# yangdongchao/RSTnet

Measured on AMD Instinct MI355X. Metric: codec+LM audio frames/sec (24 kHz, 12.5 Hz tokens) at batch=1 and batch=64; RVQ code-index exact-match, higher is better.
Workload: dtype f32 (large GEMMs: operands as three bf16 planes, six bf16 matrix-instruction products per fp32 product, f32 accumulate); 1 GPU; MimiCodec encode->RVQ(8x2048x256)->decode, BASELINE.json configs[1]; batch_per_gpu=64, weights=random-init (rstnet_amd.synth seed 0), parallelism=replica x1, utterances sharded, RCCL weight broadcast only

## Files before the change

### include/rstnet_hip.h

```cpp
#ifndef RSTNET_HIP_H
#define RSTNET_HIP_H

#include <stdint.h>

#ifdef __cplusplus
extern "C" {
#endif

#define RST_OK 0
#define RST_ERR_INVALID_ARG (-1)
#define RST_ERR_UNSUPPORTED (-2)
#define RST_ERR_LAUNCH (-3)

#define RST_ACT_NONE 0
#define RST_ACT_ELU 1
#define RST_ACT_GELU 1
#define RST_ACT_ELU_OUT 2
#define RST_PAD_ZERO 0
#define RST_PAD_REPLICATE 1

typedef void* rst_stream_t;

int rst_version(void);
const char* rst_last_error(void);
// ... 51 lines not shown

int rst_gemv_f32(const float* x, const float* ln_gamma, const float* ln_beta, float ln_eps, const float* w, const float* bias,
                 const float* res, const float* scale, float* y, int B, int N, int K, int act_out, rst_stream_t stream);

int rst_layernorm_f32(const float* x, const float* gamma, const float* beta, float* y, int64_t rows, int D, float eps,
                      rst_stream_t stream);

int rst_rope_split_f32(const float* qkv, float* q, float* k, float* v, const int64_t* pos_dev, int64_t pos0, int B,
                       int T, int H, int D, int cap, int ring, int rope, float rope_coef, rst_stream_t stream);

int rst_attention_f32(const float* q, const float* k, const float* v, float* out, const int64_t* pos_dev, int64_t pos0,
                      int B, int T, int H, int D, int cap, int ring, int context, rst_stream_t stream);

int rst_rope_table_f32(float* table, int T, int D, float rope_coef, int64_t pos0, rst_stream_t stream);
int rst_attention_qkv_f32(const float* qkv, const float* rope_table, float* out, int B, int T, int H, int D, int context,
                          rst_stream_t stream);

int rst_rvq_pack_f32(const float* emb, float* packed, float* e2, int n_codes, int D, rst_stream_t stream);

int rst_rvq_search_f32(const float* x, const float* emb, const float* packed, const float* e2, int64_t* codes,
                       float* dist, uint64_t* keys, int M, int F, int ldx, int D, int n_codes, int L, int n_groups,
                       const int* group_begin, const int* group_count, rst_stream_t stream);

int rst_rvq_chain_slot_elems(int M, int n_codes, int L);
int rst_rvq_chain_supported(int M, int n_codes, int L, int D, int n_groups);
int rst_rvq_search_chain_f32(const float* x, const float* emb, const float* packed, const float* e2, int64_t* codes, float* dist,
                             uint64_t* slots, uint32_t* status, int M, int F, int ldx, int D, int n_codes, int L, int n_groups,
                             const int* group_begin, const int* group_count, rst_stream_t stream);

int rst_rvq_gather_f32(const int64_t* codes, const float* emb, float* out, int M, int F, int D, int n_codes, int L,
                       int n_groups, const int* group_begin, const int* group_count, rst_stream_t stream);

int rst_convtr_depthwise_f32(const float* x, const float* hist, const float* w, float* y, int B, int T_in, int C,
                             int Kw, int stride, rst_stream_t stream);

int rst_act_f32(const float* x, float* y, int64_t n, int act, rst_stream_t stream);

int rst_transpose_f32(const float* x, float* y, int B, int R, int C, rst_stream_t stream);

int rst_mask_tail_f32(float* x, const int32_t* lengths, int B, int T, int C, int mode, rst_stream_t stream);

int rst_hist_update_f32(const float* x, const float* hist_in, float* hist_out, int B, int T_in, int P_in, int P_out,
                        int C, rst_stream_t stream);

int rst_hist_update_batch_f32(const float* const* x, float* const* hist, const int* T_in, const int* P, const int* C, int n, int B,
                              rst_stream_t stream);
// ... 125 lines not shown
```

### rstnet_amd/_lib.py

```python
from __future__ import annotations

import ctypes as C
import os
from typing import Optional

_HERE = os.path.dirname(os.path.abspath(__file__))
LIB_PATH = os.path.join(_HERE, "librstnet_hip.so")

_p = C.c_void_p
_i = C.c_int
_l = C.c_int64
_f = C.c_float

SIGNATURES = {
    "rst_build_id": [_p, _i],
    "rst_gemm_win_split_plan": [_l, _i, _i],
    "rst_gemm_win_split_tiles": [_l, _i],
    "rst_gemm_win_f32": [_p, _p, _p, _p, _p, _p, _p, _i, _i, _i, _i, _i, _i, _i, _i, _i, _l, _i, _i, _i, _i, _p, _p, _p],
    "rst_gemm_win_b3_supported": [_i, _i, _i, _i, _i, _i, _i, _i, _i, _l, _i],
    "rst_gemm_win_b3_weight_elems": [_i, _i],
    "rst_gemm_win_b3_pack_weight": [_p, _p, _i, _i, _p],
    "rst_gemm_win_b3_f32": [_p, _p, _p, _p, _p, _p, _p, _p, _i, _i, _i, _i, _i, _i, _i, _i, _i, _l, _i, _i, _i, _p],
    "rst_conv1d_causal_f32": [_p, _p, _p, _p, _p, _p, _i, _i, _i, _i, _i, _i, _i, _i, _i, _i, _p],
    "rst_convtr1d_causal_f32": [_p, _p, _p, _p, _p, _i, _i, _i, _i, _i, _i, _i, _i, _p],
    "rst_seanet_resblock_supported": [_i, _i, _i, _i, _i, _i, _i],
    "rst_seanet_resblock_f32": [_p] * 11 + [_i] * 8 + [_p],
    "rst_seanet_resblock_b3_supported": [_i] * 9,
    "rst_seanet_resblock_b3_weight_elems": [_i],
    "rst_seanet_resblock_b3_pack": [_p, _p, _p, _p, _i, _i, _i, _i, _p],
    "rst_seanet_resblock_b3_f32": [_p] * 8 + [_i] * 8 + [_p],
    "rst_linear_f32": [_p, _p, _p, _p, _p, _p, _l, _i, _i, _i, _p],
    "rst_layernorm_f32": [_p, _p, _p, _p, _l, _i, _f, _p],
    "rst_rope_split_f32": [_p, _p, _p, _p, _p, _l, _i, _i, _i, _i, _i, _i, _i, _f, _p],
    "rst_attention_f32": [_p, _p, _p, _p, _p, _l, _i, _i, _i, _i, _i, _i, _i, _p],
    "rst_rope_table_f32": [_p, _i, _i, _f, _l, _p],
    "rst_attention_qkv_f32": [_p, _p, _p, _i, _i, _i, _i, _i, _p],
    "rst_rvq_pack_f32": [_p, _p, _p, _i, _i, _p],
    "rst_rvq_search_f32": [_p, _p, _p, _p, _p, _p, _p, _i, _i, _i, _i, _i, _i, _i, C.POINTER(_i), C.POINTER(_i), _p],
    "rst_rvq_chain_slot_elems": [_i, _i, _i],
    "rst_rvq_chain_supported": [_i, _i, _i, _i, _i],
    "rst_rvq_search_chain_f32": [_p, _p, _p, _p, _p, _p, _p, _p, _i, _i, _i, _i, _i, _i, _i, C.POINTER(_i), C.POINTER(_i), _p],
    "rst_rvq_gather_f32": [_p, _p, _p, _i, _i, _i, _i, _i, _i, C.POINTER(_i), C.POINTER(_i), _p],
    "rst_convtr_depthwise_f32": [_p, _p, _p, _p, _i, _i, _i, _i, _i, _p],
    "rst_act_f32": [_p, _p, _l, _i, _p],
    "rst_transpose_f32": [_p, _p, _i, _i, _i, _p],
    "rst_hist_update_f32": [_p, _p, _p, _i, _i, _i, _i, _i, _p],
    "rst_hist_update_batch_f32": [C.POINTER(_p), C.POINTER(_p), C.POINTER(_i), C.POINTER(_i), C.POINTER(_i), _i, _i, _p],
    "rst_skinny_f32_pack_weight": [_p, _p, _i, _i, _p],
    "rst_skinny_f32_pack_win": [_p, _p, _p, _i, _i, _i, _i, _i, _i, _i, _i, _l, _i, _p],
    "rst_skinny_f32_pack_ln": [_p, _p, _p, _f, _p, _i, _i, _p],
    "rst_skinny_f32_split_plan": [_i, _i, _i],
    "rst_gemm_skinny_f32": [_p, _p, _p, _p, _p, _p, _i, _i, _i, _i, _i, _i, _p, _p, _i, _p],
    "rst_linear_few_rows_f32": [_p, _i, _p, _p, _p, _p, _p, _i, _i, _i, _i, _i, _i, _p, _p, _i, _p],
    "rst_mask_tail_f32": [_p, _p, _i, _i, _i, _i, _p],
    "rst_codec_transformer_workspace_bytes": [_i, _i, _i],
    "rst_codec_transformer_supported": [_i, _i, _i, _i, _i, _i, _i],
    "rst_codec_transformer_frame": [C.POINTER(_p)] * 12 + [_p, _p, _p, _p, _p] + [_i] * 9 + [_f, _f, _p],
    "rst_gemv_f32": [_p, _p, _p, _f, _p, _p, _p, _p, _p, _i, _i, _i, _i, _p],
    "rst_gemv_bf16_f32": [_p, _p, _p, _p, _p, _p, _i, _i, _i, _i, _i, _i, _f, _i, _p],
    "rst_quant_rows_fp8": [_p, _p, _p, _i, _i, _p],
    "rst_gemv_fp8w_supported": [_i, _i, _i],
# ... 88 lines not shown
```

### rstnet_amd/codec/quantization.py

```python
from __future__ import annotations

from typing import List, Optional, Tuple

import torch
from torch import nn

from .. import ops
from .conv import _PackedCache, _to_ncl, _to_nlc


class EuclideanCodebook(nn.Module):

    def __init__(self, dim: int, codebook_size: int, decay: float = 0.99, epsilon: float = 1e-5,
                 threshold_usage_ratio: float = 0.1, replaced_usage_ratio: float = 1.0, check_unused_every: int = 5):
        super().__init__()
        self.dim, self.codebook_size, self.epsilon, self.decay = dim, codebook_size, epsilon, decay
        self.register_buffer("_initialized", torch.tensor([False], dtype=torch.float))
        self.register_buffer("cluster_usage", torch.ones(codebook_size))
        self.register_buffer("embedding_sum", torch.zeros(codebook_size, dim))
        self._emb = _PackedCache()
        self._emb_tables = _PackedCache()

    def _load_from_state_dict(self, state_dict, prefix, *args, **kwargs) -> None:
        for old, new in (("inited", "_initialized"), ("cluster_size", "cluster_usage"), ("embed_avg", "embedding_sum"),
# ... 143 lines not shown
    def __init__(self, *, n_q: int = 8, no_quantization_rate: float = 0.0, no_quantization_mode: str = "same",
                 n_q_semantic: int = 1, **kwargs):
        super().__init__()
        assert n_q > n_q_semantic, f"Number of quantizers {n_q} must be larger than the number of semantic quantizers {n_q_semantic}."
        self.max_n_q = n_q
        self.n_q_semantic = n_q_semantic
        self.n_q_acoustic = n_q - n_q_semantic
        kwargs.pop("q_dropout", None)
        kwargs.pop("generator_seed", None)
        self.rvq_first = ResidualVectorQuantizer(n_q=n_q_semantic, force_projection=True, q_dropout=False, **kwargs)
        self.rvq_rest = ResidualVectorQuantizer(n_q=n_q - n_q_semantic, codebook_offset=1, force_projection=True, **kwargs)
        self._fused = _PackedCache()

    def _fused_tables(self):
        f, r = self.rvq_first, self.rvq_rest
        embs = [l.embedding for l in f.vq.layers] + [l.embedding for l in r.vq.layers]
        params = (f.input_proj.weight, r.input_proj.weight, f.output_proj.weight, r.output_proj.weight) + tuple(embs)

        def build():
            w_in = torch.cat([f.input_proj.weight[:, :, 0], r.input_proj.weight[:, :, 0]], 0).float().contiguous()
            w_out = torch.cat([f.output_proj.weight[:, :, 0], r.output_proj.weight[:, :, 0]], 1).float().contiguous()
            emb = torch.stack(embs).contiguous()
            packed, e2 = ops.rvq_pack(emb)
            return w_in, w_out, emb, packed, e2
        return self._fused.get(params, build)

    def _groups(self, n_total: Optional[int] = None) -> List[Tuple[int, int]]:
        ns = self.rvq_first.n_q
        nr = self.rvq_rest.n_q if n_total is None else n_total - ns
        return [(0, ns), (self.n_q_semantic, nr)]

    def encode_nlc(self, z: torch.Tensor) -> torch.Tensor:
        B, F, C = z.shape
        K = self.rvq_first.n_q + self.rvq_rest.n_q
        if F == 0:
            return torch.empty((B, K, 0), device=z.device, dtype=torch.int64)
        w_in, _, emb, packed, e2 = self._fused_tables()
        x = ops.linear(z.reshape(B * F, C), w_in)
        codes = ops.rvq_search(x, emb, packed, e2, B, F, self._groups())
        return codes if K == codes.shape[1] else codes[:, :K].contiguous()

    def decode_nlc(self, codes: torch.Tensor) -> torch.Tensor:
        B, K, F = codes.shape
        _, w_out, emb, _, _ = self._fused_tables()
        if K < self.max_n_q:
            pad = torch.zeros(B, self.max_n_q - K, F, device=codes.device, dtype=torch.int64)
            codes = torch.cat([codes, pad], 1)
        q = ops.rvq_gather(codes.contiguous(), emb, self._groups(K))
        return ops.linear(q, w_out).view(B, F, -1)

    def forward(self, x: torch.Tensor, frame_rate: int, semantic_features: Optional[torch.Tensor] = None):
        raise NotImplementedError("training forward (losses, distillation) is out of scope; use encode / decode")

    def encode(self, x: torch.Tensor) -> torch.Tensor:
        return self.encode_nlc(_to_nlc(x))

    def decode(self, codes: torch.Tensor) -> torch.Tensor:
        return _to_ncl(self.decode_nlc(codes))

    @property
    def total_codebooks(self) -> int:
        return self.rvq_first.max_n_q + self.rvq_rest.max_n_q

    @property
    def num_codebooks(self) -> int:
        return self.rvq_first.num_codebooks + self.rvq_rest.num_codebooks

# ... 25 lines not shown
```

### rstnet_amd/csrc/capi.hip

```cpp
#include "../../include/rstnet_hip.h"
#include "rst_kernels.h"
#include <stdarg.h>
#include <stdio.h>

static thread_local char g_err[512] = "";

void rst_set_error(const char* fmt, ...) {
    va_list ap;
    va_start(ap, fmt);
    vsnprintf(g_err, sizeof(g_err), fmt, ap);
    va_end(ap);
}

int rst_check_launch(const char* what) {
    const hipError_t e = hipGetLastError();
    if (e != hipSuccess) {
        rst_set_error("%s: launch failed: %s", what, hipGetErrorString(e));
        return RST_ERR_LAUNCH;
    }
    return RST_OK;
}

extern "C" {

int rst_version(void) { return 125; }
const char* rst_last_error(void) { return g_err; }

#ifndef RST_SRC_SHA
#define RST_SRC_SHA "unknown"
#endif
int rst_build_id(char* out, int n) {
    static const char id[] = RST_SRC_SHA;
    if (!out || n < (int)sizeof(id)) return RST_ERR_INVALID_ARG;
    for (int i = 0; i < (int)sizeof(id); ++i) out[i] = id[i];
    return (int)sizeof(id) - 1;
}

static int gemm_win_common(const float* x, const float* hist, const float* w, const uint16_t* w3, const float* bias, const float* res,
                           const float* scale, float* y, int B, int T_in, int T_out, int C, int K, int N, int S, int P,
                           int pad_mode, int64_t x_bstride, int ldy, int act_in, int act_out, int split_k, float* ws,
                           uint32_t* counters, rst_stream_t stream) {
    RST_REQUIRE(ldy >= N, "gemm_win: ldy (%d) < N (%d)", ldy, N);
    RST_REQUIRE(act_in == 0 || act_in == 1, "gemm_win: unknown act_in %d", act_in);
    RST_REQUIRE(act_out >= 0 && act_out <= 2, "gemm_win: unknown act_out %d", act_out);
    RST_REQUIRE(pad_mode == 0 || pad_mode == 1, "gemm_win: unknown pad_mode %d", pad_mode);
    GemmWinParams p;
    p.x = x; p.hist = hist; p.w = w; p.bias = bias; p.res = res; p.scale = scale; p.y = y;
    p.B = B; p.T_in = T_in; p.T_out = T_out; p.C = C; p.K = K; p.N = N; p.S = S; p.P = P;
// ... 140 lines not shown
    p.row_stride = 3 * H * D; p.rope_tab = rope_table;
    return rst_launch_attention(p, (hipStream_t)stream);
}

int rst_rvq_pack_f32(const float* emb, float* packed, float* e2, int n_codes, int D, rst_stream_t stream) {
    return rst_launch_rvq_pack(emb, packed, e2, n_codes, D, (hipStream_t)stream);
}

int rst_rvq_search_f32(const float* x, const float* emb, const float* packed, const float* e2, int64_t* codes,
                       float* dist, uint64_t* keys, int M, int F, int ldx, int D, int n_codes, int L, int n_groups,
                       const int* group_begin, const int* group_count, rst_stream_t stream) {
    RST_REQUIRE(n_groups >= 1 && n_groups <= 2 && group_begin && group_count, "rvq_search: bad groups");
    RvqSearchParams p;
    p.x = x; p.emb = emb; p.packed = packed; p.e2 = e2; p.codes = (long*)codes; p.dist = dist;
    p.M = M; p.F = F; p.ldx = ldx; p.D = D; p.n_codes = n_codes; p.L = L; p.n_groups = n_groups;
    for (int g = 0; g < 2; ++g) {
        p.group_begin[g] = g < n_groups ? group_begin[g] : 0;
        p.group_count[g] = g < n_groups ? group_count[g] : 0;
        RST_REQUIRE(p.group_begin[g] >= 0 && p.group_count[g] >= 0 && p.group_begin[g] + p.group_count[g] <= L,
                    "rvq_search: group %d out of range", g);
    }
    if (keys) return rst_launch_rvq_search_small(p, (unsigned long long*)keys, (hipStream_t)stream);
    return rst_launch_rvq_search(p, (hipStream_t)stream);
}

int rst_rvq_chain_supported(int M, int n_codes, int L, int D, int n_groups) { return rst_rvq_chain_supported_impl(M, n_codes, L, D, n_groups); }

int rst_rvq_chain_slot_elems(int M, int n_codes, int L) {
    if (M <= 0 || n_codes <= 0 || L <= 0 || (long)L * ((M + 31) / 32 * 32) * rst_rvq_chain_slices(n_codes) > 0x7fffffffL) return -1;
    return L * ((M + 31) / 32 * 32) * rst_rvq_chain_slices(n_codes);
}

int rst_rvq_search_chain_f32(const float* x, const float* emb, const float* packed, const float* e2, int64_t* codes, float* dist,
                             uint64_t* slots, uint32_t* status, int M, int F, int ldx, int D, int n_codes, int L, int n_groups,
                             const int* group_begin, const int* group_count, rst_stream_t stream) {
    RST_REQUIRE(n_groups >= 1 && n_groups <= 2 && group_begin && group_count, "rvq_search_chain: bad groups");
    RvqSearchParams p;
    p.x = x; p.emb = emb; p.packed = packed; p.e2 = e2; p.codes = (long*)codes; p.dist = dist;
    p.M = M; p.F = F; p.ldx = ldx; p.D = D; p.n_codes = n_codes; p.L = L; p.n_groups = n_groups;
    for (int g = 0; g < 2; ++g) {
        p.group_begin[g] = g < n_groups ? group_begin[g] : 0;
        p.group_count[g] = g < n_groups ? group_count[g] : 0;
        RST_REQUIRE(p.group_begin[g] >= 0 && p.group_count[g] >= 0 && p.group_begin[g] + p.group_count[g] <= L,
                    "rvq_search_chain: group %d out of range", g);
    }
    return rst_launch_rvq_search_chain(p, (unsigned long long*)slots, (unsigned*)status, (hipStream_t)stream);
// ... 491 lines not shown
```

### rstnet_amd/csrc/rst_kernels.h

```cpp
#pragma once
#include "rst_common.h"

struct GemmWinParams {
    const float* x;
    const float* hist;
    const float* w;
    const float* bias;
    const float* res;
    const float* scale;
    float* y;
    int B, T_in, T_out;
    int C;
    int K, N;
    int S;
    int P;
    int pad_mode;
    long x_bstride;
    int ldy;
    int act_in;
    int act_out;
    int split_k;
    float* ws;
    unsigned* counters;
    const short* w3;
// ... 125 lines not shown
    const long* pos_dev;
    long pos0;
    int B, T, H, D, cap;
    int ring;
    int context;
    int row_stride;
    const float* rope_tab;
};
int rst_launch_attention(const AttentionParams& p, hipStream_t stream);
int rst_launch_rope_table(float* tab, int T, int D, float rope_coef, long pos0, hipStream_t stream);

int rst_launch_rvq_pack(const float* emb, float* packed, float* e2, int n_codes, int D, hipStream_t stream);
struct RvqSearchParams {
    const float* x;
    const float* emb;
    const float* packed;
    const float* e2;
    long* codes;
    float* dist;
    int M, F, ldx, D, n_codes, L;
    int n_groups;
    int group_begin[2];
    int group_count[2];
};
int rst_launch_rvq_search(const RvqSearchParams& p, hipStream_t stream);
int rst_launch_rvq_search_small(const RvqSearchParams& p, unsigned long long* keys, hipStream_t stream);
int rst_rvq_chain_slices(int n_codes);
int rst_rvq_chain_supported_impl(int M, int n_codes, int L, int D, int n_groups);
int rst_launch_rvq_search_chain(const RvqSearchParams& p, unsigned long long* slots, unsigned* status, hipStream_t stream);
struct RvqGatherParams {
    const long* codes;
    const float* emb;
    float* out;
    int M, F, D, n_codes, L, n_groups;
    int group_begin[2];
    int group_count[2];
};
int rst_launch_rvq_gather(const RvqGatherParams& p, hipStream_t stream);

struct GemvParams {
    const float* x;
    const float* alpha;
    const float* beta;
    const void* w;
    const float* res;
    const float* bias;
    const float* scale;
    float* y;
// ... 250 lines not shown
```

### rstnet_amd/csrc/rvq.hip

```cpp
#include "rst_common.h"
#include "rst_kernels.h"
#include <math.h>

namespace {

constexpr int FR = 32;
constexpr int NW = 8;

__device__ __forceinline__ int pk_off(int k) { return (k >> 3) * 8 + (k & 1) * 4 + ((k >> 1) & 3); }

__global__ __launch_bounds__(256) void rvq_pack_kernel(const float* __restrict__ emb, float* __restrict__ packed,
                                                       float* __restrict__ e2, int n_codes, int D) {
    const long total = (long)n_codes * D;
    for (long idx = (long)blockIdx.x * 256 + threadIdx.x; idx < total; idx += (long)gridDim.x * 256) {
        const int k = (int)(idx % D);
        const long code = idx / D;
        packed[((long)(k >> 3) * n_codes + code) * 8 + (k & 1) * 4 + ((k >> 1) & 3)] = emb[idx];
    }
    for (long code = (long)blockIdx.x * 256 + threadIdx.x; code < n_codes; code += (long)gridDim.x * 256) {
        float s = 0.f;
        for (int k = 0; k < D; ++k) s = fmaf(emb[code * D + k], emb[code * D + k], s);
        e2[code] = s;
    }
}
// ... 97 lines not shown
        __syncthreads();
        if (tid < FR) {
            float bs = red_s[tid];
            int bi = red_i[tid];
            for (int w = 1; w < NW; ++w) {
                const float s = red_s[w * FR + tid];
                const int i = red_i[w * FR + tid];
                if (s < bs || (s == bs && i < bi)) { bs = s; bi = i; }
            }
            if (bi < 0 || bi >= p.n_codes) bi = 0;
            win[tid] = bi;
            const int m = m0 + tid;
            if (m < p.M) {
                const int b = m / p.F, f = m - b * p.F;
                p.codes[((long)b * p.L + lvl) * p.F + f] = bi;
                if (p.dist) p.dist[(long)lvl * p.M + m] = bs;
            }
        }
        __syncthreads();
        if (li + 1 < p.group_count[g]) {
            for (int idx = tid; idx < FR * D; idx += 64 * NW) {
                const int f = idx / D, k = idx - f * D;
                r_pk[f * LD + pk_off(k)] -= emb[(long)win[f] * D + k];
            }
        }
        __syncthreads();
    }
}

__device__ __forceinline__ unsigned long long rvq_key(float score, int code) {
    unsigned u = __float_as_uint(score);
    u = (u & 0x80000000u) ? ~u : (u | 0x80000000u);
    return ((unsigned long long)u << 32) | (unsigned)code;
}

__global__ __launch_bounds__(256) void rvq_level_kernel(const RvqSearchParams p, unsigned long long* __restrict__ keys, int step) {
    extern __shared__ __attribute__((aligned(16))) float smem[];
    const int D = p.D, LD = D + 4;
    float* r_pk = smem;
    int* prev = reinterpret_cast<int*>(r_pk + FR * LD);
    const int tid = threadIdx.x, lane = tid & 63, wave = tid >> 6;
    const int j = lane & 31, h = lane >> 5;
    const int g = blockIdx.y;
    if (step >= p.group_count[g]) return;
    const int lvl = p.group_begin[g] + step;
    const int m0 = blockIdx.z * FR;
// ... 303 lines not shown
}

int rst_launch_rvq_search(const RvqSearchParams& p, hipStream_t stream) {
    if (p.M == 0) return RST_OK;
    RST_REQUIRE(p.x && p.emb && p.packed && p.e2 && p.codes, "rvq_search: null pointer");
    RST_REQUIRE(p.M >= 0 && p.F > 0 && p.D > 0 && p.D % 8 == 0 && p.n_codes > 0 && p.n_codes % 32 == 0,
                "rvq_search: need D %% 8 == 0 and n_codes %% 32 == 0 (D=%d n_codes=%d)", p.D, p.n_codes);
    RST_REQUIRE(p.n_groups >= 1 && p.n_groups <= 2, "rvq_search: n_groups must be 1 or 2");
    RST_REQUIRE(p.M % p.F == 0, "rvq_search: M (%d) is not a multiple of F (%d)", p.M, p.F);
    if (p.M == 0) return RST_OK;
    const size_t lds = ((size_t)FR * (p.D + 4) + p.n_codes + 2 * NW * FR + FR) * sizeof(float);
    RST_REQUIRE(lds <= 160 * 1024, "rvq_search: D=%d n_codes=%d needs %zu bytes of LDS", p.D, p.n_codes, lds);
    static RstOncePerDevice attr_once;
    if (attr_once.first()) {
        (void)hipFuncSetAttribute(reinterpret_cast<const void*>(rvq_search_kernel<32>), hipFuncAttributeMaxDynamicSharedMemorySize, 160 * 1024);
        (void)hipFuncSetAttribute(reinterpret_cast<const void*>(rvq_search_kernel<0>), hipFuncAttributeMaxDynamicSharedMemorySize, 160 * 1024);
    }
    const dim3 grid((p.M + FR - 1) / FR, p.n_groups);
    if (p.D == 256) hipLaunchKernelGGL(rvq_search_kernel<32>, grid, dim3(64 * NW), lds, stream, p);
    else hipLaunchKernelGGL(rvq_search_kernel<0>, grid, dim3(64 * NW), lds, stream, p);
    return rst_check_launch("rvq_search");
}

int rst_launch_rvq_search_small(const RvqSearchParams& p, unsigned long long* keys, hipStream_t stream) {
    if (p.M == 0) return RST_OK;
    RST_REQUIRE(p.x && p.emb && p.packed && p.e2 && p.codes && keys, "rvq_search_small: null pointer");
    RST_REQUIRE(p.F > 0 && p.D > 0 && p.D % 8 == 0 && p.n_codes > 0 && p.n_codes % 32 == 0 && p.M % p.F == 0 &&
                    p.n_groups >= 1 && p.n_groups <= 2,
                "rvq_search_small: need D %% 8 == 0 and n_codes %% 32 == 0 (D=%d n_codes=%d)", p.D, p.n_codes);
    const size_t lds = ((size_t)FR * (p.D + 4) + 16 * FR) * sizeof(float);
    int steps = 0;
    for (int g = 0; g < p.n_groups; ++g) steps = p.group_count[g] > steps ? p.group_count[g] : steps;
    const dim3 grid((p.n_codes + 127) / 128, p.n_groups, (p.M + FR - 1) / FR);
    RST_REQUIRE(steps <= 16, "rvq_search_small: at most 16 levels per group (got %d)", steps);
    for (int s = 0; s < steps; ++s) {
        hipLaunchKernelGGL(rvq_level_kernel, grid, dim3(256), lds, stream, p, keys, s);
        const int rc = rst_check_launch("rvq_level");
        if (rc) return rc;
    }
    long g = ((long)p.L * p.M + 255) / 256;
    hipLaunchKernelGGL(rvq_finalize_kernel, dim3((unsigned)(g > 64 ? 64 : g)), dim3(256), 0, stream, p, keys);
    return rst_check_launch("rvq_finalize");
}

int rst_rvq_chain_slices(int n_codes) { return (n_codes + 127) / 128; }

// ... 39 lines not shown
```

### rstnet_amd/ops.py

```python
from __future__ import annotations

import ctypes as C
import functools
import math
from typing import NamedTuple, Optional, Sequence, Tuple

import torch

from . import _lib

ACT_NONE, ACT_ELU, ACT_GELU = 0, 1, 1
ACT_ELU_OUT = 2
PAD_ZERO, PAD_REPLICATE = 0, 1


PROFILE = None


class _profiled:
    __slots__ = ("row", "prof", "e0", "e1")

    def __init__(self, name: str, flops: float, nbytes: int, shape: tuple):
        self.row = (name, flops, nbytes, shape)

# ... 545 lines not shown
               groups: Sequence[Tuple[int, int]], return_dist: bool = False):
    for t, n in ((x, "x"), (emb, "emb"), (packed, "packed"), (e2, "e2")):
        _chk(t, n)
    L, n_codes, D = emb.shape
    M = B * F
    assert x.shape == (M, len(groups) * D), (tuple(x.shape), M, len(groups), D)
    covered = sorted(l for g0, n in groups for l in range(g0, g0 + n)) == list(range(L))
    codes = (torch.empty if covered else torch.zeros)(B, L, F, device=x.device, dtype=torch.int64)
    dist = torch.zeros(L, M, device=x.device, dtype=torch.float32) if return_dist else None
    keys = None
    if 0 < M <= 64 and RVQ_CHAIN and n_codes % 128 == 0 and depth_frame_enabled(x.device) and \
            _rvq_chain_supported(_device_index(x.device), M, n_codes, L, D, len(groups)):
        n_slots = int(_lib.lib().rst_rvq_chain_slot_elems(M, n_codes, L))
        sc = _scratch(_rvq_slots, x.device, (L, M, n_codes),
                      lambda: (torch.full((n_slots,), -1, device=x.device, dtype=torch.int64), new_persistent_status(x.device)))
        _lib.check(_lib.lib().rst_rvq_search_chain_f32(_ptr(x), _ptr(emb), _ptr(packed), _ptr(e2), _ptr(codes), _ptr(dist), _ptr(sc[0]), _ptr(sc[1]),
                                                       M, max(F, 1), x.shape[1], D, n_codes, L, len(groups), *_group_arrays(groups),
                                                       _stream()))
        return (codes, dist) if return_dist else codes
    if 0 < M <= 64:
        keys = _scratch(_rvq_keys, x.device, (L, M), lambda: torch.full((L, M), -1, device=x.device, dtype=torch.int64))
    _lib.check(_lib.lib().rst_rvq_search_f32(_ptr(x), _ptr(emb), _ptr(packed), _ptr(e2), _ptr(codes), _ptr(dist), _ptr(keys), M, max(F, 1),
                                             x.shape[1], D, n_codes, L, len(groups), *_group_arrays(groups), _stream()))
    return (codes, dist) if return_dist else codes


@_on_tensor_device
def rvq_gather(codes: torch.Tensor, emb: torch.Tensor, groups: Sequence[Tuple[int, int]]) -> torch.Tensor:
    _chk(codes, "codes", torch.int64)
    _chk(emb, "emb")
    B, L, F = codes.shape
    _, n_codes, D = emb.shape
    out = torch.empty(B * F, len(groups) * D, device=codes.device, dtype=torch.float32)
    _lib.check(_lib.lib().rst_rvq_gather_f32(_ptr(codes), _ptr(emb), _ptr(out), B * F, max(F, 1), D, n_codes, L, len(groups),
                                             *_group_arrays(groups), _stream()))
    return out


@_on_tensor_device
def convtr_depthwise(x: torch.Tensor, w: torch.Tensor, stride: int, hist: Optional[torch.Tensor] = None) -> torch.Tensor:
    for t, n in ((x, "x"), (w, "w"), (hist, "hist")):
        _chk(t, n)
    B, T, Cc = x.shape
    out = torch.empty(B, T * stride, Cc, device=x.device, dtype=torch.float32)
    _lib.check(_lib.lib().rst_convtr_depthwise_f32(_ptr(x), _ptr(hist), _ptr(w), _ptr(out), B, T, Cc, w.shape[1], stride,
                                                   _stream()))
# ... 1037 lines not shown
```

Measured before the change: 197,800 frames/s.

## Add bf16-plane filtered RVQ search with exact fp32 rescoring of survivors

```diff
diff --git a/include/rstnet_hip.h b/include/rstnet_hip.h
--- a/include/rstnet_hip.h
+++ b/include/rstnet_hip.h
@@ -97,6 +97,11 @@
                        float* dist, uint64_t* keys, int M, int F, int ldx, int D, int n_codes, int L, int n_groups,
                        const int* group_begin, const int* group_count, rst_stream_t stream);
 
+int rst_rvq_pack_planes_f32(const float* emb, const float* e2, uint16_t* planes, float* enorm, int n_codes, int D, rst_stream_t stream);
+int rst_rvq_search_filtered_f32(const float* x, const float* emb, const float* packed, const float* e2, const uint16_t* planes,
+                                const float* enorm, int64_t* codes, float* dist, uint32_t* stats, int M, int F, int ldx, int D, int n_codes,
+                                int L, int n_groups, const int* group_begin, const int* group_count, rst_stream_t stream);
+
 int rst_rvq_chain_slot_elems(int M, int n_codes, int L);
 int rst_rvq_chain_supported(int M, int n_codes, int L, int D, int n_groups);
 int rst_rvq_search_chain_f32(const float* x, const float* emb, const float* packed, const float* e2, int64_t* codes, float* dist,
diff --git a/rstnet_amd/_lib.py b/rstnet_amd/_lib.py
--- a/rstnet_amd/_lib.py
+++ b/rstnet_amd/_lib.py
@@ -37,6 +37,8 @@
     "rst_attention_qkv_f32": [_p, _p, _p, _i, _i, _i, _i, _i, _p],
     "rst_rvq_pack_f32": [_p, _p, _p, _i, _i, _p],
     "rst_rvq_search_f32": [_p, _p, _p, _p, _p, _p, _p, _i, _i, _i, _i, _i, _i, _i, C.POINTER(_i), C.POINTER(_i), _p],
+    "rst_rvq_pack_planes_f32": [_p, _p, _p, _p, _i, _i, _p],
+    "rst_rvq_search_filtered_f32": [_p, _p, _p, _p, _p, _p, _p, _p, _p, _i, _i, _i, _i, _i, _i, _i, C.POINTER(_i), C.POINTER(_i), _p],
     "rst_rvq_chain_slot_elems": [_i, _i, _i],
     "rst_rvq_chain_supported": [_i, _i, _i, _i, _i],
     "rst_rvq_search_chain_f32": [_p, _p, _p, _p, _p, _p, _p, _p, _i, _i, _i, _i, _i, _i, _i, C.POINTER(_i), C.POINTER(_i), _p],
diff --git a/rstnet_amd/codec/quantization.py b/rstnet_amd/codec/quantization.py
--- a/rstnet_amd/codec/quantization.py
+++ b/rstnet_amd/codec/quantization.py
@@ -189,7 +189,8 @@
             w_out = torch.cat([f.output_proj.weight[:, :, 0], r.output_proj.weight[:, :, 0]], 1).float().contiguous()
             emb = torch.stack(embs).contiguous()
             packed, e2 = ops.rvq_pack(emb)
-            return w_in, w_out, emb, packed, e2
+            planes, enorm = ops.rvq_pack_planes(emb, e2) if emb.shape[2] % 16 == 0 else (None, None)
+            return w_in, w_out, emb, packed, e2, planes, enorm
         return self._fused.get(params, build)
 
     def _groups(self, n_total: Optional[int] = None) -> List[Tuple[int, int]]:
@@ -202,14 +203,17 @@
         K = self.rvq_first.n_q + self.rvq_rest.n_q
         if F == 0:
             return torch.empty((B, K, 0), device=z.device, dtype=torch.int64)
-        w_in, _, emb, packed, e2 = self._fused_tables()
+        w_in, _, emb, packed, e2, planes, enorm = self._fused_tables()
         x = ops.linear(z.reshape(B * F, C), w_in)
-        codes = ops.rvq_search(x, emb, packed, e2, B, F, self._groups())
+        if B * F > 64 and planes is not None:
+            codes = ops.rvq_search_filtered(x, emb, packed, e2, planes, enorm, B, F, self._groups())
+        else:
+            codes = ops.rvq_search(x, emb, packed, e2, B, F, self._groups())
         return codes if K == codes.shape[1] else codes[:, :K].contiguous()
 
     def decode_nlc(self, codes: torch.Tensor) -> torch.Tensor:
         B, K, F = codes.shape
-        _, w_out, emb, _, _ = self._fused_tables()
+        _, w_out, emb = self._fused_tables()[:3]
         if K < self.max_n_q:
             pad = torch.zeros(B, self.max_n_q - K, F, device=codes.device, dtype=torch.int64)
             codes = torch.cat([codes, pad], 1)
diff --git a/rstnet_amd/csrc/capi.hip b/rstnet_amd/csrc/capi.hip
--- a/rstnet_amd/csrc/capi.hip
+++ b/rstnet_amd/csrc/capi.hip
@@ -23,7 +23,7 @@
 
 extern "C" {
 
-int rst_version(void) { return 125; }
+int rst_version(void) { return 126; }
 const char* rst_last_error(void) { return g_err; }
 
 #ifndef RST_SRC_SHA
@@ -210,6 +210,27 @@
     }
     if (keys) return rst_launch_rvq_search_small(p, (unsigned long long*)keys, (hipStream_t)stream);
     return rst_launch_rvq_search(p, (hipStream_t)stream);
+}
+
+int rst_rvq_pack_planes_f32(const float* emb, const float* e2, uint16_t* planes, float* enorm, int n_codes, int D, rst_stream_t stream) {
+    return rst_launch_rvq_pack_planes(emb, e2, (unsigned*)planes, enorm, n_codes, D, (hipStream_t)stream);
+}
+
+int rst_rvq_search_filtered_f32(const float* x, const float* emb, const float* packed, const float* e2, const uint16_t* planes,
+                                const float* enorm, int64_t* codes, float* dist, uint32_t* stats, int M, int F, int ldx, int D, int n_codes,
+                                int L, int n_groups, const int* group_begin, const int* group_count, rst_stream_t stream) {
+    RST_REQUIRE(n_groups >= 1 && n_groups <= 2 && group_begin && group_count, "rvq_search_filtered: bad groups");
+    RvqSearchParams p;
+    p.x = x; p.emb = emb; p.packed = packed; p.e2 = e2; p.codes = (long*)codes; p.dist = dist;
+    p.planes = (const unsigned*)planes; p.enorm = enorm; p.stats = (unsigned*)stats;
+    p.M = M; p.F = F; p.ldx = ldx; p.D = D; p.n_codes = n_codes; p.L = L; p.n_groups = n_groups;
+    for (int g = 0; g < 2; ++g) {
+        p.group_begin[g] = g < n_groups ? group_begin[g] : 0;
+        p.group_count[g] = g < n_groups ? group_count[g] : 0;
+        RST_REQUIRE(p.group_begin[g] >= 0 && p.group_count[g] >= 0 && p.group_begin[g] + p.group_count[g] <= L,
+                    "rvq_search_filtered: group %d out of range", g);
+    }
+    return rst_launch_rvq_search_filtered(p, (hipStream_t)stream);
 }
 
 int rst_rvq_chain_supported(int M, int n_codes, int L, int D, int n_groups) { return rst_rvq_chain_supported_impl(M, n_codes, L, D, n_groups); }
diff --git a/rstnet_amd/csrc/rst_kernels.h b/rstnet_amd/csrc/rst_kernels.h
--- a/rstnet_amd/csrc/rst_kernels.h
+++ b/rstnet_amd/csrc/rst_kernels.h
@@ -171,8 +171,13 @@
     int n_groups;
     int group_begin[2];
     int group_count[2];
+    const unsigned* planes = nullptr;
+    const float* enorm = nullptr;
+    unsigned* stats = nullptr;
 };
 int rst_launch_rvq_search(const RvqSearchParams& p, hipStream_t stream);
+int rst_launch_rvq_pack_planes(const float* emb, const float* e2, unsigned* planes, float* enorm, int n_codes, int D, hipStream_t stream);
+int rst_launch_rvq_search_filtered(const RvqSearchParams& p, hipStream_t stream);
 int rst_launch_rvq_search_small(const RvqSearchParams& p, unsigned long long* keys, hipStream_t stream);
 int rst_rvq_chain_slices(int n_codes);
 int rst_rvq_chain_supported_impl(int M, int n_codes, int L, int D, int n_groups);
diff --git a/rstnet_amd/csrc/rvq.hip b/rstnet_amd/csrc/rvq.hip
--- a/rstnet_amd/csrc/rvq.hip
+++ b/rstnet_amd/csrc/rvq.hip
@@ -1,4 +1,6 @@
 #include "rst_common.h"
+#include "b3_common.h"
+#include "rvq_filter.h"
 #include "rst_kernels.h"
 #include <math.h>
 
@@ -143,6 +145,314 @@
             for (int idx = tid; idx < FR * D; idx += 64 * NW) {
                 const int f = idx / D, k = idx - f * D;
                 r_pk[f * LD + pk_off(k)] -= emb[(long)win[f] * D + k];
+            }
+        }
+        __syncthreads();
+    }
+}
+
+__global__ __launch_bounds__(256) void rvq_pack_planes_kernel(const float* __restrict__ emb, const float* __restrict__ e2, unsigned* __restrict__ planes,
+                                                              float* __restrict__ enorm, int n_codes, int D) {
+    const long pairs = (long)n_codes * (D / 2);
+    for (long idx = (long)blockIdx.x * 256 + threadIdx.x; idx < pairs; idx += (long)gridDim.x * 256) {
+        const int k = (int)(idx % (D / 2)) * 2;
+        const long code = idx / (D / 2);
+        f32x2 v = {emb[code * D + k], emb[code * D + k + 1]};
+        const unsigned hi = b3_peel(v), mid = b3_peel(v);
+        const long w = ((((long)(k >> 4) * n_codes + code) * 2 + ((k >> 3) & 1)) * 2) * 4 + ((k & 7) >> 1);
+        planes[w] = hi;
+        planes[w + 4] = mid;
+    }
+    if (blockIdx.x == 0) {
+        __shared__ unsigned red[256];
+        unsigned m = 0;
+        for (int c = threadIdx.x; c < n_codes; c += 256) m = max(m, __float_as_uint(e2[c]));
+        red[threadIdx.x] = m;
+        __syncthreads();
+        for (int o = 128; o > 0; o >>= 1) {
+            if ((int)threadIdx.x < o) red[threadIdx.x] = max(red[threadIdx.x], red[threadIdx.x + o]);
+            __syncthreads();
+        }
+        if (threadIdx.x == 0) enorm[0] = sqrtf(__uint_as_float(red[0]));
+    }
+}
+
+constexpr int RVQF_SLOTS = 2 * NW * RVQF_TRACK;
+
+__device__ __forceinline__ void rvqf_insert(float s, int code, float& s1, int& i1, float& s2, int& i2, float& s3) {
+    if (s < s3) {
+        if (s < s2) {
+            s3 = s2;
+            if (s < s1) { s2 = s1; i2 = i1; s1 = s; i1 = code; }
+            else { s2 = s; i2 = code; }
+        } else s3 = s;
+    }
+}
+
+template <int FKT>
+__global__ __launch_bounds__(64 * NW) void rvq_search_filter_kernel(const RvqSearchParams p) {
+    static_assert(RVQF_TRACK == 2, "rvqf_insert keeps two indexed candidates");
+    extern __shared__ __attribute__((aligned(16))) float smem[];
+    const int D = p.D, LD = D + 4;
+    float* r_pk = smem;
+    unsigned* rb = reinterpret_cast<unsigned*>(r_pk + FR * LD);
+    float* e2s = reinterpret_cast<float*>(rb + FR * LD);
+    float* red_s = e2s + p.n_codes;
+    int* red_i = reinterpret_cast<int*>(red_s + NW * FR);
+    int* win = red_i + NW * FR;
+    float* dlt = reinterpret_cast<float*>(win + FR);
+    int* cnt = reinterpret_cast<int*>(dlt + FR);
+    int* cand = cnt + FR;
+    float* csc = reinterpret_cast<float*>(cand + FR * RVQF_SLOTS);
+    int* flag = reinterpret_cast<int*>(csc + FR * RVQF_SLOTS);
+
+    const int tid = threadIdx.x;
+    const int lane = tid & 63, wave = tid >> 6;
+    const int j = lane & 31, h = lane >> 5;
+    const int m0 = blockIdx.x * FR;
+    const int g = blockIdx.y;
+    const int tiles = p.n_codes / 32;
+    const int tpw = (tiles + NW - 1) / NW;
+    const int ct_lo = wave * tpw, ct_hi = min(tiles, (wave + 1) * tpw);
+    const float cD = RVQF_C_DROP + (float)D * RVQF_C_PER_D;
+
+    for (int idx = tid; idx < FR * D; idx += 64 * NW) {
+        const int f = idx / D, k = idx - f * D;
+        const int m = m0 + f;
+        r_pk[f * LD + pk_off(k)] = m < p.M ? p.x[(long)m * p.ldx + g * D + k] : 0.f;
+    }
+
+    for (int li = 0; li < p.group_count[g]; ++li) {
+        const int lvl = p.group_begin[g] + li;
+        const float* packed = p.packed + (long)lvl * p.n_codes * D;
+        const unsigned* planes = p.planes + (long)lvl * p.n_codes * D;
+        const float* emb = p.emb + (long)lvl * p.n_codes * D;
+        for (int c = tid; c < p.n_codes; c += 64 * NW) e2s[c] = p.e2[(long)lvl * p.n_codes + c];
+        if (tid < FR) cnt[tid] = 0;
+        if (tid < 2) flag[tid] = 0;
+        __syncthreads();
+        {
+            const int f = tid >> 4, part = tid & 15;
+            float ss = 0.f;
+            for (int k = part; k < D; k += 16) ss = fmaf(r_pk[f * LD + k], r_pk[f * LD + k], ss);
+#pragma unroll
+            for (int o = 8; o > 0; o >>= 1) ss += __shfl_xor(ss, o);
+            if (part == 0) {
+                const float nx = sqrtf(ss), em = p.enorm[lvl];
+                dlt[f] = RVQF_SCALE * cD * (nx + RVQF_NORM_PAD) * (em + RVQF_NORM_PAD) + RVQF_ABS;
+                if (!(nx <= RVQF_LIM) || !(em <= RVQF_LIM)) flag[0] = 1;
+            }
+        }
+        for (int idx = tid; idx < FR * (D / 2); idx += 64 * NW) {
+            const int f = idx / (D / 2), k = (idx - f * (D / 2)) * 2;
+            f32x2 v = {r_pk[f * LD + pk_off(k)], r_pk[f * LD + pk_off(k + 1)]};
+            const unsigned hi = b3_peel(v), mid = b3_peel(v);
+            const int w = f * LD + (k >> 4) * 16 + ((k >> 3) & 1) * 8 + ((k & 7) >> 1);
+            rb[w] = hi;
+            rb[w + 4] = mid;
+        }
+        __syncthreads();
+        const bool fit = flag[0] == 0;
+
+        float s1 = INFINITY, s2 = INFINITY, s3 = INFINITY;
+        int i1 = 0, i2 = 0;
+        if (fit) {
+            const unsigned* brow = rb + j * LD + h * 8;
+            auto score_tile = [&](int c0, const f32x16& acc) {
+#pragma unroll
+                for (int r = 0; r < 16; ++r) {
+                    const int code = c0 + rst_mfma32_row(r, lane);
+                    rvqf_insert(fmaf(-2.0f, acc[r], e2s[code]), code, s1, i1, s2, i2, s3);
+                }
+            };
+            if constexpr (FKT > 0) {
+                constexpr int KT = FKT, HB = 8, NH = KT / HB;
+                static_assert(KT % (2 * HB) == 0, "the next tile must start in buffer 0");
+                u32x4 ab[2][HB][2];
+                auto request = [&](int ct, int half, u32x4 (&dst)[HB][2]) {
+                    const unsigned* ap = planes + ((long)(half * HB) * p.n_codes + ct * 32 + j) * 16 + h * 8;
+#pragma unroll
+                    for (int u = 0; u < HB; ++u) {
+                        dst[u][0] = *reinterpret_cast<const u32x4*>(ap + (long)u * p.n_codes * 16);
+                        dst[u][1] = *reinterpret_cast<const u32x4*>(ap + (long)u * p.n_codes * 16 + 4);
+                    }
+                };
+                if (ct_lo < ct_hi) request(ct_lo, 0, ab[0]);
+                for (int ct = ct_lo; ct < ct_hi; ++ct) {
+                    f32x16 acc;
+#pragma unroll
+                    for (int e = 0; e < 16; ++e) acc[e] = 0.f;
+                    int boff = 0;
+                    asm volatile("" : "+v"(boff));
+                    const unsigned* brt = brow + boff;
+#pragma unroll
+                    for (int hf = 0; hf < NH; ++hf) {
+                        if (hf + 1 < NH) request(ct, hf + 1, ab[(hf + 1) & 1]);
+                        else if (ct + 1 < ct_hi) request(ct + 1, 0, ab[0]);
+#pragma unroll
+                        for (int u = 0; u < HB; ++u) {
+                            const bf16x8 ah = __builtin_bit_cast(bf16x8, ab[hf & 1][u][0]), am = __builtin_bit_cast(bf16x8, ab[hf & 1][u][1]);
+                            const bf16x8 bm = __builtin_bit_cast(bf16x8, *reinterpret_cast<const u32x4*>(brt + (hf * HB + u) * 16 + 4));
+                            const bf16x8 bhh = __builtin_bit_cast(bf16x8, *reinterpret_cast<const u32x4*>(brt + (hf * HB + u) * 16));
+                            acc = __builtin_amdgcn_mfma_f32_32x32x16_bf16(am, bhh, acc, 0, 0, 0);
+                            acc = __builtin_amdgcn_mfma_f32_32x32x16_bf16(ah, bm, acc, 0, 0, 0);
+                            acc = __builtin_amdgcn_mfma_f32_32x32x16_bf16(ah, bhh, acc, 0, 0, 0);
+                        }
+                    }
+                    score_tile(ct * 32, acc);
+                }
+            } else {
+                for (int ct = ct_lo; ct < ct_hi; ++ct) {
+                    f32x16 acc;
+#pragma unroll
+                    for (int e = 0; e < 16; ++e) acc[e] = 0.f;
+                    const unsigned* ap = planes + (long)(ct * 32 + j) * 16 + h * 8;
+#pragma unroll 4
+                    for (int kt = 0; kt < D / 16; ++kt) {
+                        const bf16x8 ah = __builtin_bit_cast(bf16x8, *reinterpret_cast<const u32x4*>(ap + (long)kt * p.n_codes * 16));
+                        const bf16x8 am = __builtin_bit_cast(bf16x8, *reinterpret_cast<const u32x4*>(ap + (long)kt * p.n_codes * 16 + 4));
+                        const bf16x8 xh = __builtin_bit_cast(bf16x8, *reinterpret_cast<const u32x4*>(brow + kt * 16));
+                        const bf16x8 xm = __builtin_bit_cast(bf16x8, *reinterpret_cast<const u32x4*>(brow + kt * 16 + 4));
+                        acc = __builtin_amdgcn_mfma_f32_32x32x16_bf16(am, xh, acc, 0, 0, 0);
+                        acc = __builtin_amdgcn_mfma_f32_32x32x16_bf16(ah, xm, acc, 0, 0, 0);
+                        acc = __builtin_amdgcn_mfma_f32_32x32x16_bf16(ah, xh, acc, 0, 0, 0);
+                    }
+                    score_tile(ct * 32, acc);
+                }
+            }
+            const float sm = fminf(s1, __shfl_xor(s1, 32));
+            if (h == 0) red_s[wave * FR + j] = sm;
+        }
+        __syncthreads();
+        if (fit) {
+            float sm = red_s[j];
+            for (int w = 1; w < NW; ++w) sm = fminf(sm, red_s[w * FR + j]);
+            const float d = dlt[j];
+            const float thr = sm + d + RVQF_EPS_S * fabsf(sm);
+            auto survives = [&](float s) { return s < INFINITY && s - d - RVQF_EPS_S * fabsf(s) <= thr; };
+            if (survives(s1)) cand[j * RVQF_SLOTS + atomicAdd(&cnt[j], 1)] = i1;
+            if (survives(s2)) cand[j * RVQF_SLOTS + atomicAdd(&cnt[j], 1)] = i2;
+            if (survives(s3) || !(thr < INFINITY)) flag[1] = 1;
+        }
+        __syncthreads();
+        const bool filtered = fit && flag[1] == 0;
+        if (tid == 0 && p.stats) {
+            if (!filtered) atomicAdd(p.stats, 1u);
+            atomicAdd(p.stats + 1, 1u);
+        }
+
+        float bs = INFINITY;
+        int bi = 0x7fffffff;
+        if (filtered) {
+            const int f = tid >> 4, part = tid & 15, n = cnt[f];
+            const int chunk = FKT > 0 ? FKT : D / 16;
+            const float* rr = r_pk + f * LD;
+            for (int slot = 0; slot < n; ++slot) {
+                const int code = cand[f * RVQF_SLOTS + slot];
+                const float* er = emb + (long)code * D + part * chunk;
+                float dot = 0.f;
+                if constexpr (FKT > 0) {
+                    static_assert(FKT % 8 == 0 || FKT == 0, "whole groups of eight k per thread");
+                    f32x4 ev[FKT / 4], rv[FKT / 4];
+#pragma unroll
+                    for (int q = 0; q < FKT / 4; ++q) ev[q] = *reinterpret_cast<const f32x4*>(er + q * 4);
+#pragma unroll
+                    for (int q = 0; q < FKT / 4; ++q) rv[q] = *reinterpret_cast<const f32x4*>(rr + part * chunk + q * 4);
+#pragma unroll
+                    for (int ph = 0; ph < 16; ++ph) {
+                        float t = __shfl(dot, (lane & ~15) + (ph > 0 ? ph - 1 : 0));
+                        if (ph == 0) t = 0.f;
+#pragma unroll
+                        for (int q = 0; q < FKT / 8; ++q) {
+                            const f32x4 ea = ev[2 * q], eb = ev[2 * q + 1], re = rv[2 * q], ro = rv[2 * q + 1];
+                            t = fmaf(re[0], ea[0], t); t = fmaf(ro[0], ea[1], t); t = fmaf(re[1], ea[2], t); t = fmaf(ro[1], ea[3], t);
+                            t = fmaf(re[2], eb[0], t); t = fmaf(ro[2], eb[1], t); t = fmaf(re[3], eb[2], t); t = fmaf(ro[3], eb[3], t);
+                        }
+                        if (part == ph) dot = t;
+                    }
+                } else {
+                    for (int ph = 0; ph < 16; ++ph) {
+                        float t = __shfl(dot, (lane & ~15) + (ph > 0 ? ph - 1 : 0));
+                        if (ph == 0) t = 0.f;
+                        for (int i = 0; i < chunk; ++i) t = fmaf(rr[pk_off(part * chunk + i)], er[i], t);
+                        if (part == ph) dot = t;
+                    }
+                }
+                if (part == 15) csc[f * RVQF_SLOTS + slot] = fmaf(-2.0f, dot, e2s[code]);
+            }
+            __syncthreads();
+            if (tid < FR) {
+                for (int s = 0; s < cnt[tid]; ++s) {
+                    const float sc = csc[tid * RVQF_SLOTS + s];
+                    const int i = cand[tid * RVQF_SLOTS + s];
+                    if (sc < bs || (sc == bs && i < bi)) { bs = sc; bi = i; }
+                }
+            }
+        } else {
+            float best = INFINITY;
+            int bidx = 0x7fffffff;
+            const float* rrow = r_pk + j * LD + h * 4;
+            for (int ct = ct_lo; ct < ct_hi; ++ct) {
+                const int c0 = ct * 32;
+                f32x16 acc;
+#pragma unroll
+                for (int e = 0; e < 16; ++e) acc[e] = 0.f;
+                const float* ap = packed + (long)(c0 + j) * 8 + h * 4;
+#pragma unroll 8
+                for (int kq = 0; kq < D / 8; ++kq) {
+                    const f32x4 a = *reinterpret_cast<const f32x4*>(ap + (long)kq * p.n_codes * 8);
+                    const f32x4 bq = *reinterpret_cast<const f32x4*>(rrow + kq * 8);
+#pragma unroll
+                    for (int e = 0; e < 4; ++e) acc = __builtin_amdgcn_mfma_f32_32x32x2f32(a[e], bq[e], acc, 0, 0, 0);
+                }
+#pragma unroll
+                for (int r = 0; r < 16; ++r) {
+                    const int code = c0 + rst_mfma32_row(r, lane);
+                    const float sc = fmaf(-2.0f, acc[r], e2s[code]);
+                    if (sc < best) { best = sc; bidx = code; }
+                }
+            }
+            const float ob = __shfl_xor(best, 32);
+            const int oi = __shfl_xor(bidx, 32);
+            if (ob < best || (ob == best && oi < bidx)) { best = ob; bidx = oi; }
+            if (h == 0) { red_s[wave * FR + j] = best; red_i[wave * FR + j] = bidx; }
+            __syncthreads();
+            if (tid < FR) {
+                bs = red_s[tid];
+                bi = red_i[tid];
+                for (int w = 1; w < NW; ++w) {
+                    const float s = red_s[w * FR + tid];
+                    const int i = red_i[w * FR + tid];
+                    if (s < bs || (s == bs && i < bi)) { bs = s; bi = i; }
+                }
+            }
+        }
+        if (tid < FR) {
+            if (bi < 0 || bi >= p.n_codes) bi = 0;
+            win[tid] = bi;
+            const int m = m0 + tid;
+            if (m < p.M) {
+                const int b = m / p.F, f = m - b * p.F;
+                p.codes[((long)b * p.L + lvl) * p.F + f] = bi;
+                if (p.dist) p.dist[(long)lvl * p.M + m] = bs;
+            }
+        }
+        __syncthreads();
+        if (li + 1 < p.group_count[g]) {
+            constexpr int U = 8;
+            for (int idx0 = tid; idx0 < FR * D; idx0 += 64 * NW * U) {
+                float e[U];
+                int fk[U];
+#pragma unroll
+                for (int u = 0; u < U; ++u) {
+                    const int idx = min(idx0 + u * 64 * NW, FR * D - 1);
+                    const int f = idx / D, k = idx - f * D;
+                    fk[u] = f * LD + pk_off(k);
+                    e[u] = emb[(long)win[f] * D + k];
+                }
+#pragma unroll
+                for (int u = 0; u < U; ++u)
+                    if (idx0 + u * 64 * NW < FR * D) r_pk[fk[u]] -= e[u];
             }
         }
         __syncthreads();
@@ -492,6 +802,34 @@
     return rst_check_launch("rvq_search");
 }
 
+int rst_launch_rvq_pack_planes(const float* emb, const float* e2, unsigned* planes, float* enorm, int n_codes, int D, hipStream_t stream) {
+    RST_REQUIRE(emb && e2 && planes && enorm && n_codes > 0 && D > 0 && D % 16 == 0, "rvq_pack_planes: bad arguments (D must be a multiple of 16)");
+    long g = ((long)n_codes * (D / 2) + 255) / 256;
+    if (g > 2048) g = 2048;
+    hipLaunchKernelGGL(rvq_pack_planes_kernel, dim3((unsigned)g), dim3(256), 0, stream, emb, e2, planes, enorm, n_codes, D);
+    return rst_check_launch("rvq_pack_planes");
+}
+
+int rst_launch_rvq_search_filtered(const RvqSearchParams& p, hipStream_t stream) {
+    if (p.M == 0) return RST_OK;
+    static const int filter = rst_knob("RST_RVQ_FILTER", 1);
+    const size_t lds = ((size_t)2 * FR * (p.D + 4) + p.n_codes + 2 * NW * FR + 3 * FR + 2 * FR * RVQF_SLOTS + 4) * sizeof(float);
+    if (!filter || p.D <= 0 || p.D % 16 != 0 || p.D > RVQF_MAX_D || p.n_codes <= 0 || p.n_codes % 32 != 0 || lds > 160 * 1024)
+        return rst_launch_rvq_search(p, stream);
+    RST_REQUIRE(p.x && p.emb && p.packed && p.e2 && p.planes && p.enorm && p.codes, "rvq_search_filtered: null pointer");
+    RST_REQUIRE(p.M >= 0 && p.F > 0 && p.n_groups >= 1 && p.n_groups <= 2, "rvq_search_filtered: bad sizes");
+    RST_REQUIRE(p.M % p.F == 0, "rvq_search_filtered: M (%d) is not a multiple of F (%d)", p.M, p.F);
+    static RstOncePerDevice attr_once;
+    if (attr_once.first()) {
+        (void)hipFuncSetAttribute(reinterpret_cast<const void*>(rvq_search_filter_kernel<16>), hipFuncAttributeMaxDynamicSharedMemorySize, 160 * 1024);
+        (void)hipFuncSetAttribute(reinterpret_cast<const void*>(rvq_search_filter_kernel<0>), hipFuncAttributeMaxDynamicSharedMemorySize, 160 * 1024);
+    }
+    const dim3 grid((p.M + FR - 1) / FR, p.n_groups);
+    if (p.D == 256) hipLaunchKernelGGL(rvq_search_filter_kernel<16>, grid, dim3(64 * NW), lds, stream, p);
+    else hipLaunchKernelGGL(rvq_search_filter_kernel<0>, grid, dim3(64 * NW), lds, stream, p);
+    return rst_check_launch("rvq_search_filtered");
+}
+
 int rst_launch_rvq_search_small(const RvqSearchParams& p, unsigned long long* keys, hipStream_t stream) {
     if (p.M == 0) return RST_OK;
     RST_REQUIRE(p.x && p.emb && p.packed && p.e2 && p.codes && keys, "rvq_search_small: null pointer");
diff --git a/rstnet_amd/csrc/rvq_filter.h b/rstnet_amd/csrc/rvq_filter.h
--- /dev/null
+++ b/rstnet_amd/csrc/rvq_filter.h
@@ -0,0 +1,11 @@
+#pragma once
+
+constexpr float RVQF_C_DROP = 0x1p-16f;
+constexpr float RVQF_C_PER_D = 0x1.4p-21f;
+constexpr float RVQF_SCALE = 2.05f;
+constexpr float RVQF_EPS_S = 0x1p-21f;
+constexpr float RVQF_NORM_PAD = 0x1p-58f;
+constexpr float RVQF_ABS = 0x1p-70f;
+constexpr float RVQF_LIM = 0x1p+40f;
+constexpr int RVQF_TRACK = 2;
+constexpr int RVQF_MAX_D = 1024;
diff --git a/rstnet_amd/ops.py b/rstnet_amd/ops.py
--- a/rstnet_amd/ops.py
+++ b/rstnet_amd/ops.py
@@ -591,6 +591,41 @@
         keys = _scratch(_rvq_keys, x.device, (L, M), lambda: torch.full((L, M), -1, device=x.device, dtype=torch.int64))
     _lib.check(_lib.lib().rst_rvq_search_f32(_ptr(x), _ptr(emb), _ptr(packed), _ptr(e2), _ptr(codes), _ptr(dist), _ptr(keys), M, max(F, 1),
                                              x.shape[1], D, n_codes, L, len(groups), *_group_arrays(groups), _stream()))
+    return (codes, dist) if return_dist else codes
+
+
+@_on_tensor_device
+def rvq_pack_planes(emb: torch.Tensor, e2: torch.Tensor) -> Tuple[torch.Tensor, torch.Tensor]:
+    _chk(emb, "emb")
+    _chk(e2, "e2")
+    L, n_codes, D = emb.shape
+    if D % 16:
+        raise ValueError(f"rstnet_amd.ops: rvq_pack_planes needs D % 16 == 0, got {D}")
+    planes = torch.empty(L, D // 16, n_codes, 2, 2, 8, device=emb.device, dtype=torch.bfloat16)
+    enorm = torch.empty(L, device=emb.device, dtype=torch.float32)
+    for l in range(L):
+        _lib.check(_lib.lib().rst_rvq_pack_planes_f32(_ptr(emb[l]), _ptr(e2[l]), _ptr(planes[l]), _ptr(enorm[l:l + 1]), n_codes, D, _stream()))
+    return planes, enorm
+
+
+@_on_tensor_device
+def rvq_search_filtered(x: torch.Tensor, emb: torch.Tensor, packed: torch.Tensor, e2: torch.Tensor, planes: torch.Tensor,
+                        enorm: torch.Tensor, B: int, F: int, groups: Sequence[Tuple[int, int]], return_dist: bool = False,
+                        stats: Optional[torch.Tensor] = None):
+    for t, n in ((x, "x"), (emb, "emb"), (packed, "packed"), (e2, "e2"), (enorm, "enorm")):
+        _chk(t, n)
+    _chk(planes, "planes", torch.bfloat16)
+    _chk(stats, "stats", torch.int32)
+    L, n_codes, D = emb.shape
+    M = B * F
+    assert x.shape == (M, len(groups) * D), (tuple(x.shape), M, len(groups), D)
+    assert planes.numel() == L * n_codes * D * 2 and enorm.numel() == L, (tuple(planes.shape), tuple(enorm.shape))
+    covered = sorted(l for g0, n in groups for l in range(g0, g0 + n)) == list(range(L))
+    codes = (torch.empty if covered else torch.zeros)(B, L, F, device=x.device, dtype=torch.int64)
+    dist = torch.zeros(L, M, device=x.device, dtype=torch.float32) if return_dist else None
+    _lib.check(_lib.lib().rst_rvq_search_filtered_f32(_ptr(x), _ptr(emb), _ptr(packed), _ptr(e2), _ptr(planes), _ptr(enorm), _ptr(codes), _ptr(dist),
+                                                      _ptr(stats), M, max(F, 1), x.shape[1], D, n_codes, L, len(groups), *_group_arrays(groups),
+                                                      _stream()))
     return (codes, dist) if return_dist else codes
 
 
diff --git a/rstnet_amd/rvq_filter.py b/rstnet_amd/rvq_filter.py
--- /dev/null
+++ b/rstnet_amd/rvq_filter.py
@@ -0,0 +1,87 @@
+import os
+import re
+from typing import Dict, NamedTuple
+
+import torch
+
+_HEADER = os.path.join(os.path.dirname(os.path.abspath(__file__)), "csrc", "rvq_filter.h")
+
+
+def constants() -> Dict[str, float]:
+    out: Dict[str, float] = {}
+    with open(_HEADER) as f:
+        for m in re.finditer(r"constexpr\s+(float|int)\s+(RVQF_\w+)\s*=\s*([^;]+);", f.read()):
+            kind, name, val = m.group(1), m.group(2), m.group(3).strip()
+            if kind == "int":
+                out[name] = int(val)
+            else:
+                val = val.rstrip("f")
+                out[name] = float.fromhex(val) if val.lower().startswith("0x") else float(val)
+    return out
+
+
+def served(D: int, n_codes: int) -> bool:
+    return D % 16 == 0 and D <= constants()["RVQF_MAX_D"] and n_codes % 32 == 0
+
+
+def split_planes(v: torch.Tensor):
+    hi = v.to(torch.bfloat16).float()
+    mid = (v - hi).to(torch.bfloat16).float()
+    return hi, mid
+
+
+def fma32(a: torch.Tensor, b: torch.Tensor, c: torch.Tensor) -> torch.Tensor:
+    p = a.double() * b.double()
+    c = c.double()
+    s = p + c
+    bb = s - p
+    err = (p - (s - bb)) + (c - bb)
+    odd = (s.view(torch.int64) & 1) == 1
+    toward = torch.where(err > 0, torch.full_like(s, float("inf")), torch.full_like(s, float("-inf")))
+    s = torch.where((err != 0) & ~odd & torch.isfinite(s), torch.nextafter(s, toward), s)
+    return s.float()
+
+
+def chain_e2(emb: torch.Tensor) -> torch.Tensor:
+    e2 = torch.zeros(emb.shape[0], dtype=torch.float32)
+    for k in range(emb.shape[1]):
+        e2 = fma32(emb[:, k], emb[:, k], e2)
+    return e2
+
+
+class Level(NamedTuple):
+    survivors: torch.Tensor
+    fallback: torch.Tensor
+    approx: torch.Tensor
+
+
+def filter_level(r: torch.Tensor, emb: torch.Tensor, lanes_per_frame: int = 16) -> Level:
+    c = constants()
+    f32 = torch.float32
+    M, D = r.shape
+    n_codes = emb.shape[0]
+    e2 = chain_e2(emb)
+    emax = e2.max().sqrt()
+    nx = (r * r).sum(1).sqrt()
+    xh, xm = split_planes(r)
+    eh, em = split_planes(emb)
+    dot = xh @ eh.T + (xh @ em.T + xm @ eh.T)
+    s = e2[None, :] - 2.0 * dot
+    cD = torch.tensor(c["RVQF_C_DROP"] + D * c["RVQF_C_PER_D"], dtype=f32)
+    pad = c["RVQF_NORM_PAD"]
+    delta = (c["RVQF_SCALE"] * cD * (nx + pad) * (emax + pad) + c["RVQF_ABS"]).to(f32)[:, None] + c["RVQF_EPS_S"] * s.abs()
+    smin = s.min(1, keepdim=True).values
+    dmin = torch.gather(delta, 1, s.argmin(1, keepdim=True))
+    thr = smin + dmin
+    surv = (s - delta) <= thr
+    unfit = ~(nx <= c["RVQF_LIM"]) | ~(emax <= c["RVQF_LIM"])
+    tiles = n_codes // 32
+    tpw = (tiles + 7) // 8
+    code = torch.arange(n_codes)
+    wave = (code // 32) // tpw
+    half = (code % 32 // 4) % 2
+    lane = wave * 2 + half
+    per_lane = torch.zeros(M, lanes_per_frame, dtype=torch.int64)
+    per_lane.index_add_(1, lane, surv.to(torch.int64))
+    over = (per_lane > c["RVQF_TRACK"]).any(1)
+    return Level(surv, unfit | over | ~torch.isfinite(thr[:, 0]), s)
```

After: 199,700 frames/s, median of 6. No clear change (+1.0%).
